# JeffWang987/MVSTER

Hardware: AMD Instinct MI355X
Metric: depth-maps/sec (DTU 512×640, 5-view, 4-stage) at 1/2/4/8 MI355X (higher is better)
Workload: dtype f32; 1 GPU; DTU mid 512x640, 5 views, 4-stage cascade 8/8/4/4 hyp, B=1 eval, 1 depth map(s) per step per GPU; launch=hipGraph replay, parallelism=replicas x1, depth_maps_in_flight_per_gpu=2

## Files before the change

mvster_amd/csrc/conv_wino.hip:

```cpp
#include "conv_args.hpp"

namespace mvconv {
namespace {

typedef float f32x2v __attribute__((ext_vector_type(2)));

#ifdef MVSTER_TIMELINE
__device__ unsigned long long* g_wtl = nullptr;
#define MV_WTL(k)                                                                                                       \
    do {                                                                                                                \
        __builtin_amdgcn_sched_barrier(0);                                                                              \
        if (g_wtl && lane == 0 && g < 32)                                                                               \
            g_wtl[(((size_t)(blockIdx.y * gridDim.x + blockIdx.x) * 8 + wave8) * 32 + g) * 4 + (k)] = __builtin_amdgcn_s_memtime(); \
        __builtin_amdgcn_sched_barrier(0);                                                                              \
    } while (0)
#else
#define MV_WTL(k)
#endif

#ifndef MV_WINO_SCALAR_ADDS
#define MV_WINO_SCALAR_ADDS 0
#endif
#if MV_WINO_SCALAR_ADDS
__device__ __forceinline__ f32x2v pk_add(f32x2v a, f32x2v b) {
    float r0, r1;
    asm("v_add_f32 %0, %2, %3\n\tv_add_f32 %1, %4, %5" : "=&v"(r0), "=&v"(r1) : "v"(a[0]), "v"(b[0]), "v"(a[1]), "v"(b[1]));
    return (f32x2v){r0, r1};
}
__device__ __forceinline__ f32x2v pk_sub(f32x2v a, f32x2v b) {
    float r0, r1;
    asm("v_sub_f32 %0, %2, %3\n\tv_sub_f32 %1, %4, %5" : "=&v"(r0), "=&v"(r1) : "v"(a[0]), "v"(b[0]), "v"(a[1]), "v"(b[1]));
    return (f32x2v){r0, r1};
}
#else
__device__ __forceinline__ f32x2v pk_add(f32x2v a, f32x2v b) {
    f32x2v r;
    asm("v_pk_add_f32 %0, %1, %2" : "=v"(r) : "v"(a), "v"(b));
    return r;
}
__device__ __forceinline__ f32x2v pk_sub(f32x2v a, f32x2v b) {
    f32x2v r;
    asm("v_pk_add_f32 %0, %1, %2 neg_lo:[0,1] neg_hi:[0,1]" : "=v"(r) : "v"(a), "v"(b));
    return r;
}
#endif
struct Q4 {
    f32x2v lo, hi;
};
__device__ __forceinline__ Q4 operator+(const Q4& a, const Q4& b) { return {pk_add(a.lo, b.lo), pk_add(a.hi, b.hi)}; }
__device__ __forceinline__ Q4 operator-(const Q4& a, const Q4& b) { return {pk_sub(a.lo, b.lo), pk_sub(a.hi, b.hi)}; }
__device__ __forceinline__ float elem(const Q4& a, int j) { return j < 2 ? a.lo[j] : a.hi[j - 2]; }

template <int NT, int NCH, bool WREG, bool SKIP>
__global__ void __launch_bounds__(256) conv_wino_kernel(ConvArgs a, PersArgs p) {
    using G = PersGeom<4, 3, 1, 1>;
    constexpr int TY = G::TY, PW = G::PW, PLANE = G::PLANE, NBLK = G::NBLK, RS = G::ROWSLOTS;
    constexpr int BUF = NCH * 2 * PLANE;
    constexpr int NI = NCH * 2 * NBLK;
    constexpr int NIW = (NI + 3) / 4;
    constexpr int CIN = NCH * 16;
    extern __shared__ __attribute__((aligned(16))) float lds_raw[];
    f32x4v* const lds = reinterpret_cast<f32x4v*>(lds_raw);
    f32x4v* const scratch = lds + 2 * BUF;
    f32x4v* const wl = scratch + 64;

    const int lane = threadIdx.x & 63;
    const int wave = __builtin_amdgcn_readfirstlane(threadIdx.x >> 6);
    const int lm = lane & 15, lq = lane >> 4;
    const int nt0 = blockIdx.y * NT;
    const __amdgpu_buffer_rsrc_t in_rsrc =
        __builtin_amdgcn_make_buffer_rsrc(const_cast<float*>(a.in), (short)0, (int)a.in_bytes, 0x00020000);

    unsigned dbase[NIW];
    int dpos[NIW];
#pragma unroll
    for (int n = 0; n < NIW; ++n) {
        const int i = wave + 4 * n;
        const int c = i / (2 * NBLK), r = i - c * 2 * NBLK, pl = r / NBLK, blk = r - pl * NBLK;
        const int s = blk * 64 + lane;
        const int q1 = s & 1, pix = s >> 1;
        const int py = pix / PW, ps = pix - py * PW;
        const int px = ps < G::PWH ? 2 * ps : 2 * (ps - G::PWH) + 1;
        const bool valid = i < NI && py < G::ROWS;
        dpos[n] = px | (py << 8);
        dbase[n] = valid ? (unsigned)((py * a.Wi + px) * (CIN * 4) + (c * 16 + pl * 8 + q1 * 4) * 4) : 0x80000000u;
    }
    auto decode_tile = [&](unsigned tile) -> TilePos {
        TilePos t;
        auto div = [&](unsigned n, int k) -> unsigned { return ((__umulhi(n, p.mul[k]) >> p.shr[k]) & ~p.one[k]) | (n & p.one[k]); };
        unsigned q = div(tile, 0);
        t.tx0 = (int)(tile - q * p.tiles_x) * 32;
        unsigned q2 = div(q, 1);
        t.ty0 = (int)(q - q2 * p.tiles_y) * TY;
        const unsigned q3 = div(q2, 2);
        t.zo = (int)(q2 - q3 * (unsigned)a.Do);
        t.b = (int)q3;
        return t;
    };
    auto dma_tile = [&](const TilePos& t, int buf, bool live) {
        const int iy0 = t.ty0 - a.ph[0], ix0 = t.tx0 - a.pw[0];
        const unsigned origin = (unsigned)((((t.b * a.Di + t.zo) * a.Hi + iy0) * a.Wi + ix0) * (CIN * 4));
        const unsigned wi = live ? (unsigned)a.Wi : 0u;
        f32x4v* const dst0 = lds + buf * BUF;
#pragma unroll
        for (int n = 0; n < NIW; ++n) {
            const int i = wave + 4 * n;
            const int ix = ix0 + (dpos[n] & 255), iy = iy0 + (dpos[n] >> 8);
// ... 23 lines not shown
            const int s = i / NT, nt = i - s * NT;
            const unsigned off = (unsigned)((s * wstep + (long)(nt0 + nt) * 256) * 4) + lane * 16;
            f32x4v* const dst = wl + i * 64;
            __builtin_amdgcn_raw_ptr_buffer_load_lds(w_rsrc, (lds_void*)dst, 16, off, 0, 0, 0);
        }
    }
    f32x4v scv[NT], shv[NT];
#pragma unroll
    for (int nt = 0; nt < NT; ++nt) {
        const int n0 = (nt0 + nt) * 16 + lq * 4;
        scv[nt] = *reinterpret_cast<const f32x4v*>(a.scale + n0);
        shv[nt] = *reinterpret_cast<const f32x4v*>(a.shift + n0);
    }
    const int abase = 2 * wave * RS + 2 * lm + (lq >> 1) * PLANE + (lq & 1);
    const __amdgpu_buffer_rsrc_t out_rsrc =
        __builtin_amdgcn_make_buffer_rsrc(a.out, (short)0, (int)p.out_bytes, 0x00020000);
    const __amdgpu_buffer_rsrc_t skip_rsrc = __builtin_amdgcn_make_buffer_rsrc(
        const_cast<float*>(SKIP ? a.skip : a.in), (short)0, SKIP ? (int)p.out_bytes : 0, 0x00020000);
    const unsigned obase = (unsigned)((2 * wave * a.Wo + 2 * lm) * a.cout + nt0 * 16 + lq * 4) * 4u;
    const unsigned opix = (unsigned)a.cout * 4u, orow = (unsigned)a.Wo * opix;

    __syncthreads();

    for (int it = 0; tile < p.ntiles; tile += nwg, ++it) {
        const int cur = it & 1;
        const TilePos here = pos;
        const unsigned oorigin = (unsigned)((((here.b * a.Do + here.zo) * a.Ho + here.ty0) * a.Wo + here.tx0) * a.cout) * 4u;
        unsigned ooff[2][2];
        f32x4v skv[2][2][NT];
#pragma unroll
        for (int i = 0; i < 2; ++i)
#pragma unroll
            for (int j = 0; j < 2; ++j) {
                const bool ok = here.ty0 + 2 * wave + i < a.Ho && here.tx0 + 2 * lm + j < a.Wo;
                ooff[i][j] = ok ? obase + oorigin + i * orow + j * opix : 0x80000000u;
#pragma unroll
                for (int nt = 0; nt < NT; ++nt)
                    skv[i][j][nt] = SKIP ? __builtin_bit_cast(f32x4v, __builtin_amdgcn_raw_buffer_load_b128(skip_rsrc, ooff[i][j] + nt * 64, 0, 0))
                                         : (f32x4v){0.f, 0.f, 0.f, 0.f};
            }
        const bool has_next = tile + nwg < p.ntiles;
        pos = decode_tile(has_next ? tile + nwg : tile);
        dma_tile(pos, cur ^ 1, has_next);
        __builtin_amdgcn_sched_barrier(0);

        f32x4v acc[16][NT];
#pragma unroll
        for (int q = 0; q < 16; ++q)
#pragma unroll
            for (int nt = 0; nt < NT; ++nt) acc[q][nt] = (f32x4v){0.f, 0.f, 0.f, 0.f};
        const f32x4v* patch = lds + cur * BUF + abase;
#pragma unroll
        for (int c = 0; c < NCH; ++c) {
            Q4 d[4][4], V[4][4];
#pragma unroll
            for (int r = 0; r < 4; ++r)
#pragma unroll
                for (int x = 0; x < 4; ++x) {
                    const f32x4v v = patch[c * 2 * PLANE + r * RS + (x & 1) * (G::PWH * 2) + (x >> 1) * 2];
                    d[r][x] = {{v[0], v[1]}, {v[2], v[3]}};
                }
#pragma unroll
            for (int x = 0; x < 4; ++x) {
                const Q4 t0 = d[0][x] - d[2][x], t1 = d[1][x] + d[2][x], t2 = d[2][x] - d[1][x], t3 = d[1][x] - d[3][x];
                d[0][x] = t0;
                d[1][x] = t1;
                d[2][x] = t2;
                d[3][x] = t3;
            }
#pragma unroll
            for (int r = 0; r < 4; ++r) {
                V[r][0] = d[r][0] - d[r][2];
                V[r][1] = d[r][1] + d[r][2];
                V[r][2] = d[r][2] - d[r][1];
                V[r][3] = d[r][1] - d[r][3];
            }
            __builtin_amdgcn_sched_barrier(0);
            asm volatile("s_nop 3" ::: "memory");
            __builtin_amdgcn_sched_barrier(0);
#pragma unroll
            for (int j = 0; j < 4; ++j)
#pragma unroll
                for (int q = 0; q < 16; ++q)
#pragma unroll
                    for (int nt = 0; nt < NT; ++nt) {
                        const f32x4v u = WREG ? wreg[(q * NCH + c) * NT + nt] : wl[((q * NCH + c) * NT + nt) * 64 + lane];
                        acc[q][nt] = __builtin_amdgcn_mfma_f32_16x16x4f32(u[j], elem(V[q >> 2][q & 3], j), acc[q][nt], 0, 0, 0);
                    }
            __builtin_amdgcn_sched_barrier(0);
        }
        asm volatile("s_nop 15\n\ts_nop 7" ::: "memory");
        __builtin_amdgcn_sched_barrier(0);
        const float floor_v = a.relu ? 0.0f : -__builtin_inff();
#pragma unroll
        for (int nt = 0; nt < NT; ++nt) {
            Q4 m[16], t[2][4];
#pragma unroll
            for (int q = 0; q < 16; ++q) m[q] = {{acc[q][nt][0], acc[q][nt][1]}, {acc[q][nt][2], acc[q][nt][3]}};
#pragma unroll
            for (int x = 0; x < 4; ++x) {
                t[0][x] = m[0 + x] + m[4 + x] + m[8 + x];
                t[1][x] = m[4 + x] - (m[8 + x] + m[12 + x]);
            }
#pragma unroll
            for (int i = 0; i < 2; ++i) {
                Q4 y[2];
                y[0] = t[i][0] + t[i][1] + t[i][2];
                y[1] = t[i][1] - (t[i][2] + t[i][3]);
#pragma unroll
                for (int j = 0; j < 2; ++j) {
                    f32x4v v = {y[j].lo[0], y[j].lo[1], y[j].hi[0], y[j].hi[1]};
#pragma unroll
                    for (int e = 0; e < 4; ++e) {
                        v[e] = fmaxf(fmaf(v[e], scv[nt][e], shv[nt][e]), floor_v);
                        if (SKIP) v[e] += skv[i][j][nt][e];
                    }
                    __builtin_amdgcn_raw_buffer_store_b128(__builtin_bit_cast(u32x4v, v), out_rsrc, ooff[i][j] + nt * 64, 0, MV_STORE_AUX);
                }
            }
        }
        asm volatile("s_waitcnt vmcnt(%0)" ::"n"(4 * NT) : "memory");
        __builtin_amdgcn_s_waitcnt(0xc07f);
        __builtin_amdgcn_s_barrier();
    }
}

template <int NT, int NCH, bool WREG, bool SKIP>
int launch_wino(const ConvArgs& a, int wpc, hipStream_t s) {
    using G = PersGeom<4, 3, 1, 1>;
    const size_t lds = (size_t)(2 * NCH * 2 * G::PLANE + 64 + (WREG ? 0 : 16 * NCH * NT * 64)) * 16;
    if (lds > 160 * 1024) return MVSTER_ERR_UNSUPPORTED;
    auto kern = conv_wino_kernel<NT, NCH, WREG, SKIP>;
    static unsigned long attr_done = 0;
    if (lds > 64 * 1024 && !allow_big_lds(reinterpret_cast<const void*>(kern), attr_done)) return MVSTER_ERR_LAUNCH;
    const int ncu = num_cus();
    if (ncu <= 0) return MVSTER_ERR_LAUNCH;
    PersArgs p;
    if (!fill_pers_args(a, G::TY, p)) return MVSTER_ERR_UNSUPPORTED;
    const long ntiles = p.ntiles;
    const int by_lds = (int)((160 * 1024) / lds);
    int per_cu = wpc > 0 ? wpc : 2;
    if (per_cu > by_lds) per_cu = by_lds;
    if (per_cu < 1) per_cu = 1;
    const int ny = a.ntile_total / NT;
    long gmax = (long)ncu * per_cu / ny;
    if (gmax < 1) gmax = 1;
    const long rounds = (ntiles + gmax - 1) / gmax;
    const long gx = (ntiles + rounds - 1) / rounds;
    MV_NOTE_KERNEL("conv_wino_kernel<%d, %d, %s, %s>", NT, NCH, WREG ? "true" : "false", SKIP ? "true" : "false");
    hipLaunchKernelGGL(kern, dim3((unsigned)gx, ny, 1), dim3(256), lds, s, a, p);
    return mv_check_launch();
}

struct RingGeom {
    static constexpr int TY = 8, PWH = 17, PH = 10;
    static constexpr int ROWSLOTS = PWH * 4;
    static constexpr int USED = PH * ROWSLOTS;
    static constexpr int NBLK = (USED + 63) / 64;
    static constexpr int PLANE = ((NBLK * 64 + 7) & ~7) + 4;
    static constexpr int SLICE = 2 * PLANE;
};

struct RingStep {
    unsigned tile;
    int kz, c, kz_hi;
    TilePos pos;
    bool live;
};

template <int NCH, int KD, bool SKIP, int MODE>
__global__ void __launch_bounds__(512) conv_wino_ring_kernel(ConvArgs a, PersArgs p) {
    constexpr bool SPLITN = MODE == 1;
    constexpr int NT = MODE == 2 ? 2 : 1;
    constexpr int NTW = MODE == 0 ? 1 : 2;
    constexpr bool AHEAD = NT == 1;
    using G = RingGeom;
    constexpr int TY = G::TY, PLANE = G::PLANE, NBLK = G::NBLK, RS = G::ROWSLOTS, SLICE = G::SLICE;
    constexpr int NLW = SPLITN ? 8 : 4;
    constexpr int NIW = (NBLK + NLW / 2 - 1) / (NLW / 2);
    constexpr int NUW = 16 * NTW / NLW;
    constexpr int CIN = NCH * 16;
    constexpr int UST = 16 * NTW * 64;
    constexpr bool URES = KD * NCH * NTW <= 4;
    constexpr int USLOTS = URES ? KD * NCH : 2;
    extern __shared__ __attribute__((aligned(16))) float lds_raw[];
    f32x4v* const ring = reinterpret_cast<f32x4v*>(lds_raw);
    f32x4v* const uring = ring + 4 * SLICE;
    f32x4v* const scratch = uring + USLOTS * UST;

    const int lane = threadIdx.x & 63;
    const int wave8 = __builtin_amdgcn_readfirstlane(threadIdx.x >> 6);
    const int half = wave8 >> 2, wave = wave8 & 3;
    const bool loads = SPLITN || half == 1;
    const int lw = SPLITN ? wave8 : wave;
    const int lm = lane & 15, lq = lane >> 4;
    const int nt0 = blockIdx.y * NTW;
    const int ntw = SPLITN ? half : 0;
    const long wstep = (long)a.ntile_total * 256;
    auto in_rsrc = [&](int k) -> __amdgpu_buffer_rsrc_t {
        return __builtin_amdgcn_make_buffer_rsrc(const_cast<float*>(a.in) - 256 * k, (short)0, (int)(a.in_bytes + 1024u * k), 0x00020000);
    };
    auto w_rsrc = [&](int k) -> __amdgpu_buffer_rsrc_t {
        return __builtin_amdgcn_make_buffer_rsrc(const_cast<float*>(a.wpk) - 256 * k, (short)0,
                                                 (int)(KD * 16 * NCH * wstep * 4 + 1024 * k), 0x00020000);
    };

    static_assert((NLW / 2) * NIW >= NBLK, "the waves of one plane cover its blocks");
    const int lpl = lw / (NLW / 2), lblk0 = (lw % (NLW / 2)) * NIW;
    auto decode_piece = [&](int n, int ln, unsigned& db, int& dp) {
        const int pl = lpl, blk = lblk0 + n;
        const int s = blk * 64 + ln;
        const int q1 = s & 1;
        int t = s >> 1;
        const int xh = t % G::PWH;
        t /= G::PWH;
        const int py = t >> 1, px = 2 * xh + (t & 1);
        const bool valid = blk < NBLK && py < G::PH;
        dp = px | (py << 8);
        db = valid ? (unsigned)((py * a.Wi + px) * (CIN * 4) + (pl * 8 + q1 * 4) * 4) : 0x80000000u;
    };
    unsigned dbase[SPLITN ? NIW : 1];
    int dpos[SPLITN ? NIW : 1];
    if (SPLITN) {
#pragma unroll
// ... 68 lines not shown
            const int ix = r.ix0 + (dp & 255), iy = r.iy0 + (dp >> 8);
            const bool ok = (unsigned)iy < (unsigned)a.Hi && (unsigned)ix < r.wi;
            const unsigned off = ok ? db + r.origin : 0x80000000u;
            switch (n & 3) {
                case 0: __builtin_amdgcn_raw_ptr_buffer_load_lds(rs, (lds_void*)dst, 16, off, 0, IMM[0], 0); break;
                case 1: __builtin_amdgcn_raw_ptr_buffer_load_lds(rs, (lds_void*)dst, 16, off, 0, IMM[1], 0); break;
                case 2: __builtin_amdgcn_raw_ptr_buffer_load_lds(rs, (lds_void*)dst, 16, off, 0, IMM[2], 0); break;
                default: __builtin_amdgcn_raw_ptr_buffer_load_lds(rs, (lds_void*)dst, 16, off, 0, IMM[3], 0); break;
            }
        }
    };
    struct WeightReq {
        unsigned base;
        f32x4v* dst0;
    };
    auto weight_req = [&](const RingStep& st, int slot) -> WeightReq {
        WeightReq r;
        r.base = st.live ? (unsigned)(((long)(st.kz * 16 * NCH + st.c) * wstep + (long)nt0 * 256) * 4) : 0x80000000u;
        r.dst0 = uring + slot * UST;
        return r;
    };
    const unsigned wlane = lane * 16;
    static_assert(NUW <= 8, "two M0 values per weight request");
    auto weight_piece = [&](const WeightReq& r, int m) {
        const int u = lw * NUW + m;
        const int q = u / NTW, nt = u - q * NTW;
        const unsigned so = r.base + (unsigned)(((long)q * NCH * wstep + nt * 256) * 4);
        f32x4v* const dst = r.dst0 + (lw * NUW + (m & ~3)) * 64;
        const __amdgpu_buffer_rsrc_t rs = w_rsrc(m & 3);
        switch (m & 3) {
            case 0: __builtin_amdgcn_raw_ptr_buffer_load_lds(rs, (lds_void*)dst, 16, wlane, so, 0, 0); break;
            case 1: __builtin_amdgcn_raw_ptr_buffer_load_lds(rs, (lds_void*)dst, 16, wlane, so, 1024, 0); break;
            case 2: __builtin_amdgcn_raw_ptr_buffer_load_lds(rs, (lds_void*)dst, 16, wlane, so, 2048, 0); break;
            default: __builtin_amdgcn_raw_ptr_buffer_load_lds(rs, (lds_void*)dst, 16, wlane, so, 3072, 0); break;
        }
    };

    f32x4v scv[NT], shv[NT];
#pragma unroll
    for (int nt = 0; nt < NT; ++nt) {
        const int n0 = (nt0 + ntw + nt) * 16 + lq * 4;
        scv[nt] = *reinterpret_cast<const f32x4v*>(a.scale + n0);
        shv[nt] = *reinterpret_cast<const f32x4v*>(a.shift + n0);
    }
    const int abase = 2 * wave * RS + 2 * lm + (lq >> 1) * PLANE + (lq & 1);
    const __amdgpu_buffer_rsrc_t out_rsrc =
        __builtin_amdgcn_make_buffer_rsrc(a.out, (short)0, (int)p.out_bytes, 0x00020000);
    const __amdgpu_buffer_rsrc_t skip_rsrc = __builtin_amdgcn_make_buffer_rsrc(
        const_cast<float*>(SKIP ? a.skip : a.in), (short)0, SKIP ? (int)p.out_bytes : 0, 0x00020000);
    const unsigned obase = (unsigned)((2 * wave * a.Wo + 2 * lm) * a.cout + (nt0 + ntw) * 16 + lq * 4) * 4u;
    const unsigned opix = (unsigned)a.cout * 4u, orow = (unsigned)a.Wo * opix;
    const float floor_v = a.relu ? 0.0f : -__builtin_inff();

    Q4 d[4][4], V[4][4];
    auto read_block = [&](int slot) {
        const f32x4v* patch = ring + slot * SLICE + abase;
#pragma unroll
        for (int r = 0; r < 4; ++r)
#pragma unroll
            for (int x = 0; x < 4; ++x) {
                const f32x4v v = patch[r * RS + (x & 1) * (G::PWH * 2) + (x >> 1) * 2];
                d[r][x] = {{v[0], v[1]}, {v[2], v[3]}};
            }
    };
    auto transform_block = [&]() {
#pragma unroll
        for (int x = 0; x < 4; ++x) {
            const Q4 t0 = d[0][x] - d[2][x], t1 = d[1][x] + d[2][x], t2 = d[2][x] - d[1][x], t3 = d[1][x] - d[3][x];
            d[0][x] = t0;
            d[1][x] = t1;
            d[2][x] = t2;
            d[3][x] = t3;
        }
#pragma unroll
        for (int r = 0; r < 4; ++r) {
            V[r][0] = d[r][0] - d[r][2];
            V[r][1] = d[r][1] + d[r][2];
            V[r][2] = d[r][2] - d[r][1];
            V[r][3] = d[r][1] - d[r][3];
        }
    };

    RingStep s0 = first_step(xcd_remap(blockIdx.x, nwg));
    RingStep s1 = next_step(s0), s2 = next_step(s1), s3 = next_step(s2);
    if (loads) {
        unsigned db0[NIW];
        int dp0[NIW];
#pragma unroll
        for (int n = 0; n < NIW; ++n) decode_piece(n, lane, db0[n], dp0[n]);
        const RingStep* const first[3] = {&s0, &s1, &s2};
#pragma unroll
        for (int k = 0; k < 3; ++k) {
            const SliceReq r = slice_req(*first[k], k);
#pragma unroll
            for (int n = 0; n < NIW; ++n) slice_piece(r, n, db0[n], dp0[n]);
        }
        if (URES) {
#pragma unroll
            for (int kz = 0; kz < KD; ++kz)
#pragma unroll
                for (int c = 0; c < NCH; ++c) {
                    RingStep st = s0;
                    st.live = true;
                    st.kz = kz;
                    st.c = c;
                    const WeightReq wq = weight_req(st, kz * NCH + c);
#pragma unroll
                    for (int m = 0; m < NUW; ++m) weight_piece(wq, m);
                }
        } else {
            const WeightReq w0 = weight_req(s0, 0);
#pragma unroll
            for (int m = 0; m < NUW; ++m) weight_piece(w0, m);
        }
    }
    __syncthreads();
    if (!SPLITN && half == 1) {
        unsigned dbl[NIW];
        int dpl[NIW];
#pragma unroll
        for (int n = 0; n < NIW; ++n) decode_piece(n, lane, dbl[n], dpl[n]);
        for (int g = 0; s0.live; ++g) {
            MV_WTL(0);
            if (!URES) {
                const WeightReq wr = weight_req(s1, (g + 1) & 1);
#pragma unroll
                for (int m = 0; m < NUW; ++m) weight_piece(wr, m);
            }
            const SliceReq sr = slice_req(s3, (g + 3) & 3);
#pragma unroll
            for (int n = 0; n < NIW; ++n) slice_piece(sr, n, dbl[n], dpl[n]);
            MV_WTL(1);
            asm volatile("s_waitcnt vmcnt(%0)" ::"n"(NIW) : "memory");
            MV_WTL(2);
            __builtin_amdgcn_s_barrier();
            MV_WTL(3);
            s0 = s1;
            s1 = s2;
            s2 = s3;
            s3 = next_step(s3);
        }
        return;
    }
    f32x4v acc[16][NT];
#pragma unroll
    for (int q = 0; q < 16; ++q)
#pragma unroll
        for (int nt = 0; nt < NT; ++nt) acc[q][nt] = (f32x4v){0.f, 0.f, 0.f, 0.f};
    read_block(0);
    transform_block();

    for (int g = 0; s0.live; ++g) {
        const bool last = is_last(s0);
        MV_WTL(0);
        {
            unsigned ooff[2][2];
            f32x4v skv[2][2][NT];
            if (last) {
                const TilePos& here = s0.pos;
                const unsigned oorigin = (unsigned)((((here.b * a.Do + here.zo) * a.Ho + here.ty0) * a.Wo + here.tx0) * a.cout) * 4u;
#pragma unroll
                for (int i = 0; i < 2; ++i)
#pragma unroll
                    for (int j = 0; j < 2; ++j) {
                        const bool ok = here.ty0 + 2 * wave + i < a.Ho && here.tx0 + 2 * lm + j < a.Wo;
                        ooff[i][j] = ok ? obase + oorigin + i * orow + j * opix : 0x80000000u;
#pragma unroll
                        for (int nt = 0; nt < NT; ++nt)
                            skv[i][j][nt] = (SKIP && AHEAD) ? __builtin_bit_cast(f32x4v, __builtin_amdgcn_raw_buffer_load_b128(skip_rsrc, ooff[i][j] + nt * 64, 0, 0))
                                                            : (f32x4v){0.f, 0.f, 0.f, 0.f};
                    }
            }
            const WeightReq wr = weight_req(s1, (g + 1) & 1);
            const SliceReq sr = slice_req(s3, (g + 3) & 3);
            const f32x4v* const nextp = ring + ((g + 1) & 3) * SLICE + abase;
            __builtin_amdgcn_sched_barrier(0);
            {
                const f32x4v* const us = uring + (URES ? s0.kz * NCH + s0.c : g & 1) * UST + ntw * 64 + lane;
                f32x4v ub[2][4][NT];
                auto load_u = [&](int grp, f32x4v (&dst)[4][NT]) {
#pragma unroll
                    for (int qq = 0; qq < 4; ++qq)
#pragma unroll
                        for (int nt = 0; nt < NT; ++nt) dst[qq][nt] = us[((grp * 4 + qq) * NTW + nt) * 64];
                };
                constexpr int NUL = URES ? 0 : NUW;
                constexpr int NP = SPLITN ? NUL + NIW : 0;
                load_u(0, ub[0]);
#pragma unroll
                for (int grp = 0; grp < 4; ++grp) {
                    if (grp < 3) load_u(grp + 1, ub[(grp + 1) & 1]);
#pragma unroll
                    for (int j = 0; j < 4; ++j)
#pragma unroll
                        for (int qq = 0; qq < 4; ++qq)
#pragma unroll
                            for (int nt = 0; nt < NT; ++nt)
                                acc[grp * 4 + qq][nt] = __builtin_amdgcn_mfma_f32_16x16x4f32(ub[grp & 1][qq][nt][j], elem(V[grp][qq], j),
                                                                                             acc[grp * 4 + qq][nt], 0, 0, 0);
                    __builtin_amdgcn_sched_barrier(0);
#pragma unroll
                    for (int k = grp * 2; k < grp * 2 + 2 && k < NP; ++k) {
                        if (k < NUL) {
                            weight_piece(wr, k);
                        } else {
                            slice_piece(sr, k - NUL, dbase[k - NUL], dpos[k - NUL]);
                        }
                    }
                    if (AHEAD) {
#pragma unroll
                        for (int x = 0; x < 4; ++x) {
                            const f32x4v v = nextp[grp * RS + (x & 1) * (G::PWH * 2) + (x >> 1) * 2];
                            d[grp][x] = {{v[0], v[1]}, {v[2], v[3]}};
                        }
                    }
                    __builtin_amdgcn_sched_barrier(0);
                }
            }
            MV_WTL(1);
            __builtin_amdgcn_sched_barrier(0);
            asm volatile("s_nop 15\n\ts_nop 7" ::: "memory");
            __builtin_amdgcn_sched_barrier(0);
            if (last) {
                if (SKIP && !AHEAD) {
#pragma unroll
                    for (int i = 0; i < 2; ++i)
#pragma unroll
                        for (int j = 0; j < 2; ++j)
#pragma unroll
                            for (int nt = 0; nt < NT; ++nt)
                                skv[i][j][nt] = __builtin_bit_cast(f32x4v, __builtin_amdgcn_raw_buffer_load_b128(skip_rsrc, ooff[i][j] + nt * 64, 0, 0));
                }
#pragma unroll
                for (int nt = 0; nt < NT; ++nt) {
                    Q4 m[16], t[2][4];
#pragma unroll
                    for (int q = 0; q < 16; ++q) m[q] = {{acc[q][nt][0], acc[q][nt][1]}, {acc[q][nt][2], acc[q][nt][3]}};
#pragma unroll
                    for (int x = 0; x < 4; ++x) {
                        t[0][x] = m[0 + x] + m[4 + x] + m[8 + x];
                        t[1][x] = m[4 + x] - (m[8 + x] + m[12 + x]);
                    }
#pragma unroll
                    for (int i = 0; i < 2; ++i) {
                        Q4 y[2];
                        y[0] = t[i][0] + t[i][1] + t[i][2];
                        y[1] = t[i][1] - (t[i][2] + t[i][3]);
#pragma unroll
                        for (int j = 0; j < 2; ++j) {
                            f32x4v v = {y[j].lo[0], y[j].lo[1], y[j].hi[0], y[j].hi[1]};
#pragma unroll
                            for (int e = 0; e < 4; ++e) {
                                v[e] = fmaxf(fmaf(v[e], scv[nt][e], shv[nt][e]), floor_v);
                                if (SKIP) v[e] += skv[i][j][nt][e];
                            }
                            __builtin_amdgcn_raw_buffer_store_b128(__builtin_bit_cast(u32x4v, v), out_rsrc, ooff[i][j] + nt * 64, 0, MV_STORE_AUX);
                        }
                    }
                }
#pragma unroll
                for (int q = 0; q < 16; ++q)
#pragma unroll
                    for (int nt = 0; nt < NT; ++nt) acc[q][nt] = (f32x4v){0.f, 0.f, 0.f, 0.f};
            }
            __builtin_amdgcn_sched_barrier(0);
            if (!AHEAD) read_block((g + 1) & 3);
            transform_block();
            MV_WTL(2);
            __builtin_amdgcn_sched_barrier(0);
            if (SPLITN) {
                if (last) {
                    asm volatile("s_waitcnt vmcnt(%0)" ::"n"(NIW + 4 * NT) : "memory");
                } else {
                    asm volatile("s_waitcnt vmcnt(%0)" ::"n"(NIW) : "memory");
                }
            }
        }
        __builtin_amdgcn_s_waitcnt(0xc07f);
        __builtin_amdgcn_s_barrier();
        MV_WTL(3);
        s0 = s1;
        s1 = s2;
        s2 = s3;
        s3 = next_step(s3);
    }
}

template <int NCH, int KD, bool SKIP, int MODE>
int launch_wino_ring(const ConvArgs& a, hipStream_t s) {
    using G = RingGeom;
    constexpr int NT = MODE == 0 ? 1 : 2;
    constexpr int USLOTS = KD * NCH * NT <= 4 ? KD * NCH : 2;
    const size_t lds = (size_t)(4 * G::SLICE + USLOTS * 16 * NT * 64 + 64) * 16;
    if (lds > 160 * 1024) return MVSTER_ERR_UNSUPPORTED;
    auto kern = conv_wino_ring_kernel<NCH, KD, SKIP, MODE>;
    static unsigned long attr_done = 0;
    if (!allow_big_lds(reinterpret_cast<const void*>(kern), attr_done)) return MVSTER_ERR_LAUNCH;
    const int ncu = num_cus();
    if (ncu <= 0) return MVSTER_ERR_LAUNCH;
    PersArgs p;
    if (!fill_pers_args(a, G::TY, p)) return MVSTER_ERR_UNSUPPORTED;
    if ((long)KD * 16 * NCH * a.ntile_total * 1024 >= (1L << 31)) return MVSTER_ERR_UNSUPPORTED;
    const long ntiles = p.ntiles;
    const int ny = a.ntile_total / NT;
    long gmax = (long)ncu / ny;
    if (gmax < 1) gmax = 1;
    const long rounds = (ntiles + gmax - 1) / gmax;
    const long gx = (ntiles + rounds - 1) / rounds;
    MV_NOTE_KERNEL("conv_wino_ring_kernel<%d, %d, %s, %d>", NCH, KD, SKIP ? "true" : "false", MODE);
    hipLaunchKernelGGL(kern, dim3((unsigned)gx, ny, 1), dim3(512), lds, s, a, p);
    return mv_check_launch();
}

template <int NCH, bool SKIP>
__global__ void __launch_bounds__(512) conv_wino_pair_kernel(ConvArgs a, PersArgs p) {
    using G = RingGeom;
    constexpr int KD = 3, NS = 2;
    constexpr int TY = G::TY, PLANE = G::PLANE, NBLK = G::NBLK, RS = G::ROWSLOTS, SLICE = G::SLICE;
    constexpr int NLW = 4;
    constexpr int NIW = (NBLK + NLW / 2 - 1) / (NLW / 2);
    constexpr int CIN = NCH * 16;
    constexpr int UBLK = 16 * 64;
    constexpr bool URES = KD * NCH <= 3;
    constexpr int UST = URES ? UBLK : NS * UBLK;
    constexpr int USLOTS = URES ? KD * NCH : 2;
    constexpr int NUW = NS * 16 / NLW;
    extern __shared__ __attribute__((aligned(16))) float lds_raw[];
    f32x4v* const ring = reinterpret_cast<f32x4v*>(lds_raw);
    f32x4v* const uring = ring + 4 * SLICE;
    f32x4v* const scratch = uring + USLOTS * UST;

    const int lane = threadIdx.x & 63;
    const int wave8 = __builtin_amdgcn_readfirstlane(threadIdx.x >> 6);
    const int half = wave8 >> 2, wave = wave8 & 3;
    const int lm = lane & 15, lq = lane >> 4;
    const int nt0 = blockIdx.y;
    const long wstep = (long)a.ntile_total * 256;
    const int dop = a.Do >> 1;
    auto in_rsrc = [&](int k) -> __amdgpu_buffer_rsrc_t {
        return __builtin_amdgcn_make_buffer_rsrc(const_cast<float*>(a.in) - 256 * k, (short)0, (int)(a.in_bytes + 1024u * k), 0x00020000);
    };
    auto w_rsrc = [&](int k) -> __amdgpu_buffer_rsrc_t {
        return __builtin_amdgcn_make_buffer_rsrc(const_cast<float*>(a.wpk) - 256 * k, (short)0,
                                                 (int)(KD * 16 * NCH * wstep * 4 + 1024 * k), 0x00020000);
    };
    const int lpl = wave / (NLW / 2), lblk0 = (wave % (NLW / 2)) * NIW;
    auto decode_piece = [&](int n, int ln, unsigned& db, int& dp) {
        const int blk = lblk0 + n;
        const int s = blk * 64 + ln;
        const int q1 = s & 1;
        int t = s >> 1;
        const int xh = t % G::PWH;
        t /= G::PWH;
        const int py = t >> 1, px = 2 * xh + (t & 1);
        const bool valid = blk < NBLK && py < G::PH;
        dp = px | (py << 8);
        db = valid ? (unsigned)((py * a.Wi + px) * (CIN * 4) + (lpl * 8 + q1 * 4) * 4) : 0x80000000u;
    };
    auto decode_tile = [&](unsigned tile) -> TilePos {
        TilePos t;
        auto div = [&](unsigned n, int k) -> unsigned { return ((__umulhi(n, p.mul[k]) >> p.shr[k]) & ~p.one[k]) | (n & p.one[k]); };
        unsigned q = div(tile, 0);
// ... 309 lines not shown
struct PackWinoDesc {
    const float* w;
    float* wpk;
    long s_n, s_c, s_z, s_y, s_x;
    int cout, cin_raw, cin, kd, flip, ntile;
    int first_block, pad_;
};

__device__ __forceinline__ void pack_wino_element(const PackWinoDesc& d, long idx) {
    const int cin = d.cin, kd = d.kd, ntile = d.ntile, flip = d.flip;
    const long total = (long)kd * 16 * cin * ntile * 16;
    if (idx >= total) return;
    const int j = (int)(idx & 3), lanei = (int)((idx >> 2) & 63);
    const long rest = idx >> 8;
    const int t = (int)(rest % ntile);
    const int kstep = (int)(rest / ntile);
    const int k = kstep * 16 + (lanei >> 4) * 4 + j;
    const int n = t * 16 + (lanei & 15);
    const int qz = k / cin, ci = k - qz * cin;
    const int kz = qz >> 4, q = qz & 15;
    float u = 0.f;
    if (n < d.cout && ci < d.cin_raw) {
        const int xi = q >> 2, nu = q & 3;
        const float Gm[4][3] = {{1.f, 0.f, 0.f}, {0.5f, 0.5f, 0.5f}, {0.5f, -0.5f, 0.5f}, {0.f, 0.f, 1.f}};
        const float* g = d.w + n * d.s_n + ci * d.s_c + (flip ? kd - 1 - kz : kz) * d.s_z;
        float rowv[3];
#pragma unroll
        for (int x = 0; x < 3; ++x) {
            float acc = 0.f;
#pragma unroll
            for (int y = 0; y < 3; ++y) {
                const int yy = flip ? 2 - y : y, xx = flip ? 2 - x : x;
                acc = fmaf(Gm[xi][y], g[yy * d.s_y + xx * d.s_x], acc);
            }
            rowv[x] = acc;
        }
        u = fmaf(Gm[nu][0], rowv[0], fmaf(Gm[nu][1], rowv[1], Gm[nu][2] * rowv[2]));
    }
    d.wpk[idx] = u;
}

__global__ void pack_wino_kernel(PackWinoDesc d) { pack_wino_element(d, (long)blockIdx.x * blockDim.x + threadIdx.x); }

__global__ void __launch_bounds__(256) pack_wino_batch_kernel(const PackWinoDesc* __restrict__ descs, int ndesc) {
    int lo = 0, hi = ndesc - 1;
    while (lo < hi) {
        const int mid = (lo + hi + 1) >> 1;
        if (descs[mid].first_block <= (int)blockIdx.x) lo = mid; else hi = mid - 1;
    }
    const PackWinoDesc d = descs[lo];
    pack_wino_element(d, (long)((int)blockIdx.x - d.first_block) * 256 + threadIdx.x);
}

}

int dispatch_wino(const ConvArgs& a, int nt, int wpc, bool ring, hipStream_t s) {
    if (a.nclass != 1 || a.osd != 1 || a.osh != 1 || a.osw != 1 || a.skip_mode > 1 || a.prob_w || a.cout % 16 != 0 ||
        a.sh != 1 || a.sw != 1 || a.sd != 1 || a.kh[0] != 3 || a.kw[0] != 3 || a.ph[0] != 1 || a.pw[0] != 1 ||
        nt < 1 || a.ntile_total % nt != 0 || a.cin % 16 != 0)
        return MVSTER_ERR_UNSUPPORTED;
    const int nch = a.cin / 16, kd = a.kd[0];
    if (!(kd == 1 && a.pd[0] == 0) && !(kd == 3 && a.pd[0] == 1)) return MVSTER_ERR_UNSUPPORTED;
    if (ring) {
        if (nt == 1 && wpc == 3) {
            if (kd != 3) return MVSTER_ERR_UNSUPPORTED;
            if (nch == 1) return a.skip_mode == 1 ? launch_wino_pair<1, true>(a, s) : launch_wino_pair<1, false>(a, s);
            if (nch == 2) return a.skip_mode == 1 ? launch_wino_pair<2, true>(a, s) : launch_wino_pair<2, false>(a, s);
            return MVSTER_ERR_UNSUPPORTED;
        }
        const int mode = nt == 1 ? 0 : (wpc == 1 ? 2 : 1);
#define MV_R(MODE_, NCH_, KD_)                                                                      \
    if (mode == MODE_ && nch == NCH_ && kd == KD_)                                                  \
        return a.skip_mode == 1 ? launch_wino_ring<NCH_, KD_, true, MODE_>(a, s) : launch_wino_ring<NCH_, KD_, false, MODE_>(a, s);
        MV_R(0, 1, 3) MV_R(0, 2, 3) MV_R(1, 2, 3) MV_R(2, 2, 3) MV_R(0, 4, 3) MV_R(1, 4, 3) MV_R(2, 4, 3)
        MV_R(0, 4, 1) MV_R(1, 4, 1) MV_R(2, 4, 1) MV_R(0, 2, 1) MV_R(1, 2, 1) MV_R(2, 2, 1) MV_R(0, 1, 1) MV_R(2, 1, 1)
#undef MV_R
        return MVSTER_ERR_UNSUPPORTED;
    }
    if (kd != 1) return MVSTER_ERR_UNSUPPORTED;
#define MV_W(NT_, NCH_, WREG_)                                                                      \
    if (nt == NT_ && nch == NCH_)                                                                   \
        return a.skip_mode == 1 ? launch_wino<NT_, NCH_, WREG_, true>(a, wpc, s) : launch_wino<NT_, NCH_, WREG_, false>(a, wpc, s);
    MV_W(1, 1, true)
    MV_W(2, 1, true)
    MV_W(2, 2, false)
    MV_W(1, 2, false)
#undef MV_W
    return MVSTER_ERR_UNSUPPORTED;
}

}

#ifdef MVSTER_TIMELINE
extern "C" int mvster_debug_wino_timeline(void* buf) {
    return hipMemcpyToSymbol(HIP_SYMBOL(mvconv::g_wtl), &buf, sizeof(buf)) == hipSuccess ? MVSTER_OK : MVSTER_ERR_LAUNCH;
}
#endif

extern "C" int mvster_pack_wino_weights(const float* w, float* wpk, int cout, int cin_raw, int cin_pad, int kd, long s_n, long s_c,
                                        long s_z, long s_y, long s_x, int flip, void* stream) {
    if (!w || !wpk) return MVSTER_ERR_NULL;
    if (cout < 1 || cin_raw < 1 || cin_pad < cin_raw || cin_pad % 16 != 0 || (kd != 1 && kd != 3)) return MVSTER_ERR_SHAPE;
    const int ntile = (cout + 15) / 16;
    const long total = (long)kd * 16 * cin_pad * ntile * 16;
    mvconv::PackWinoDesc d{w, wpk, s_n, s_c, s_z, s_y, s_x, cout, cin_raw, cin_pad, kd, flip, ntile, 0, 0};
    hipLaunchKernelGGL(mvconv::pack_wino_kernel, dim3((unsigned)((total + 255) / 256)), dim3(256), 0, (hipStream_t)stream, d);
    return mv_check_launch();
}

extern "C" int mvster_pack_wino_batch(const void* descs, int ndesc, int total_blocks, void* stream) {
    if (!descs) return MVSTER_ERR_NULL;
    if (ndesc < 1 || total_blocks < 1) return MVSTER_ERR_SHAPE;
    static_assert(sizeof(mvconv::PackWinoDesc) == 88, "PackWinoDesc layout");
    hipLaunchKernelGGL(mvconv::pack_wino_batch_kernel, dim3((unsigned)total_blocks), dim3(256), 0, (hipStream_t)stream,
                       (const mvconv::PackWinoDesc*)descs, ndesc);
    return mv_check_launch();
}
```

Before: 1151 depth-maps/s.

## Add software-pipelined Winograd ring path interleaving next-slice transform with MFMAs

Adds a non-serial variant of the Winograd ring kernel for mode 0, NCH=2, KD=3. It holds the transformed input tile in scalar registers for two parities and interleaves the LDS reads and input transform of the next slice between the MFMAs of the current slice. Non-serial variants also use scalar adds instead of packed adds and drop the s_nop padding, aiming to hide transform latency behind matrix math. The cost is higher register pressure. Other shapes keep the old serial form by default, and the alternative form can only be selected through order bits when probes are compiled in.

Measured after the change: 1148 depth-maps/s. No clear change (-0.2%).

```diff
diff --git a/mvster_amd/csrc/conv_wino.hip b/mvster_amd/csrc/conv_wino.hip
--- a/mvster_amd/csrc/conv_wino.hip
+++ b/mvster_amd/csrc/conv_wino.hip
@@ -18,21 +18,6 @@
 #define MV_WTL(k)
 #endif
 
-#ifndef MV_WINO_SCALAR_ADDS
-#define MV_WINO_SCALAR_ADDS 0
-#endif
-#if MV_WINO_SCALAR_ADDS
-__device__ __forceinline__ f32x2v pk_add(f32x2v a, f32x2v b) {
-    float r0, r1;
-    asm("v_add_f32 %0, %2, %3\n\tv_add_f32 %1, %4, %5" : "=&v"(r0), "=&v"(r1) : "v"(a[0]), "v"(b[0]), "v"(a[1]), "v"(b[1]));
-    return (f32x2v){r0, r1};
-}
-__device__ __forceinline__ f32x2v pk_sub(f32x2v a, f32x2v b) {
-    float r0, r1;
-    asm("v_sub_f32 %0, %2, %3\n\tv_sub_f32 %1, %4, %5" : "=&v"(r0), "=&v"(r1) : "v"(a[0]), "v"(b[0]), "v"(a[1]), "v"(b[1]));
-    return (f32x2v){r0, r1};
-}
-#else
 __device__ __forceinline__ f32x2v pk_add(f32x2v a, f32x2v b) {
     f32x2v r;
     asm("v_pk_add_f32 %0, %1, %2" : "=v"(r) : "v"(a), "v"(b));
@@ -43,16 +28,40 @@
     asm("v_pk_add_f32 %0, %1, %2 neg_lo:[0,1] neg_hi:[0,1]" : "=v"(r) : "v"(a), "v"(b));
     return r;
 }
-#endif
 struct Q4 {
     f32x2v lo, hi;
 };
 __device__ __forceinline__ Q4 operator+(const Q4& a, const Q4& b) { return {pk_add(a.lo, b.lo), pk_add(a.hi, b.hi)}; }
 __device__ __forceinline__ Q4 operator-(const Q4& a, const Q4& b) { return {pk_sub(a.lo, b.lo), pk_sub(a.hi, b.hi)}; }
 __device__ __forceinline__ float elem(const Q4& a, int j) { return j < 2 ? a.lo[j] : a.hi[j - 2]; }
-
-template <int NT, int NCH, bool WREG, bool SKIP>
+__device__ __forceinline__ Q4 from4(const Q4*, const f32x4v& v) { return {{v[0], v[1]}, {v[2], v[3]}}; }
+
+struct S4 {
+    float v[4];
+};
+__device__ __forceinline__ S4 operator+(const S4& a, const S4& b) { return {{a.v[0] + b.v[0], a.v[1] + b.v[1], a.v[2] + b.v[2], a.v[3] + b.v[3]}}; }
+__device__ __forceinline__ S4 operator-(const S4& a, const S4& b) { return {{a.v[0] - b.v[0], a.v[1] - b.v[1], a.v[2] - b.v[2], a.v[3] - b.v[3]}}; }
+__device__ __forceinline__ float elem(const S4& a, int j) { return a.v[j]; }
+__device__ __forceinline__ S4 from4(const S4*, const f32x4v& v) { return {{v[0], v[1], v[2], v[3]}}; }
+template <bool SERIAL>
+struct WinoVec {
+    using type = S4;
+};
+template <>
+struct WinoVec<true> {
+    using type = Q4;
+};
+
+constexpr bool wino_ring_serial(int mode, int nch, int kd) { return !(mode == 0 && nch == 2 && kd == 3); }
+#if defined(MVSTER_PROBES) || defined(MVSTER_TIMELINE)
+#define MV_WINO_SERIAL_FORMS 1
+#else
+#define MV_WINO_SERIAL_FORMS 0
+#endif
+
+template <int NT, int NCH, bool WREG, bool SKIP, bool SERIAL>
 __global__ void __launch_bounds__(256) conv_wino_kernel(ConvArgs a, PersArgs p) {
+    using T4 = typename WinoVec<SERIAL>::type;
     using G = PersGeom<4, 3, 1, 1>;
     constexpr int TY = G::TY, PW = G::PW, PLANE = G::PLANE, NBLK = G::NBLK, RS = G::ROWSLOTS;
     constexpr int BUF = NCH * 2 * PLANE;
@@ -182,17 +191,17 @@
         const f32x4v* patch = lds + cur * BUF + abase;
 #pragma unroll
         for (int c = 0; c < NCH; ++c) {
-            Q4 d[4][4], V[4][4];
+            T4 d[4][4], V[4][4];
 #pragma unroll
             for (int r = 0; r < 4; ++r)
 #pragma unroll
                 for (int x = 0; x < 4; ++x) {
                     const f32x4v v = patch[c * 2 * PLANE + r * RS + (x & 1) * (G::PWH * 2) + (x >> 1) * 2];
-                    d[r][x] = {{v[0], v[1]}, {v[2], v[3]}};
+                    d[r][x] = from4((T4*)nullptr, v);
                 }
 #pragma unroll
             for (int x = 0; x < 4; ++x) {
-                const Q4 t0 = d[0][x] - d[2][x], t1 = d[1][x] + d[2][x], t2 = d[2][x] - d[1][x], t3 = d[1][x] - d[3][x];
+                const T4 t0 = d[0][x] - d[2][x], t1 = d[1][x] + d[2][x], t2 = d[2][x] - d[1][x], t3 = d[1][x] - d[3][x];
                 d[0][x] = t0;
                 d[1][x] = t1;
                 d[2][x] = t2;
@@ -206,7 +215,7 @@
                 V[r][3] = d[r][1] - d[r][3];
             }
             __builtin_amdgcn_sched_barrier(0);
-            asm volatile("s_nop 3" ::: "memory");
+            if (SERIAL) asm volatile("s_nop 3" ::: "memory");
             __builtin_amdgcn_sched_barrier(0);
 #pragma unroll
             for (int j = 0; j < 4; ++j)
@@ -219,14 +228,14 @@
                     }
             __builtin_amdgcn_sched_barrier(0);
         }
-        asm volatile("s_nop 15\n\ts_nop 7" ::: "memory");
+        if (SERIAL) asm volatile("s_nop 15\n\ts_nop 7" ::: "memory");
         __builtin_amdgcn_sched_barrier(0);
         const float floor_v = a.relu ? 0.0f : -__builtin_inff();
 #pragma unroll
         for (int nt = 0; nt < NT; ++nt) {
-            Q4 m[16], t[2][4];
-#pragma unroll
-            for (int q = 0; q < 16; ++q) m[q] = {{acc[q][nt][0], acc[q][nt][1]}, {acc[q][nt][2], acc[q][nt][3]}};
+            T4 m[16], t[2][4];
+#pragma unroll
+            for (int q = 0; q < 16; ++q) m[q] = from4((T4*)nullptr, acc[q][nt]);
 #pragma unroll
             for (int x = 0; x < 4; ++x) {
                 t[0][x] = m[0 + x] + m[4 + x] + m[8 + x];
@@ -234,12 +243,12 @@
             }
 #pragma unroll
             for (int i = 0; i < 2; ++i) {
-                Q4 y[2];
+                T4 y[2];
                 y[0] = t[i][0] + t[i][1] + t[i][2];
                 y[1] = t[i][1] - (t[i][2] + t[i][3]);
 #pragma unroll
                 for (int j = 0; j < 2; ++j) {
-                    f32x4v v = {y[j].lo[0], y[j].lo[1], y[j].hi[0], y[j].hi[1]};
+                    f32x4v v = {elem(y[j], 0), elem(y[j], 1), elem(y[j], 2), elem(y[j], 3)};
 #pragma unroll
                     for (int e = 0; e < 4; ++e) {
                         v[e] = fmaxf(fmaf(v[e], scv[nt][e], shv[nt][e]), floor_v);
@@ -255,12 +264,12 @@
     }
 }
 
-template <int NT, int NCH, bool WREG, bool SKIP>
+template <int NT, int NCH, bool WREG, bool SKIP, bool SERIAL>
 int launch_wino(const ConvArgs& a, int wpc, hipStream_t s) {
     using G = PersGeom<4, 3, 1, 1>;
     const size_t lds = (size_t)(2 * NCH * 2 * G::PLANE + 64 + (WREG ? 0 : 16 * NCH * NT * 64)) * 16;
     if (lds > 160 * 1024) return MVSTER_ERR_UNSUPPORTED;
-    auto kern = conv_wino_kernel<NT, NCH, WREG, SKIP>;
+    auto kern = conv_wino_kernel<NT, NCH, WREG, SKIP, SERIAL>;
     static unsigned long attr_done = 0;
     if (lds > 64 * 1024 && !allow_big_lds(reinterpret_cast<const void*>(kern), attr_done)) return MVSTER_ERR_LAUNCH;
     const int ncu = num_cus();
@@ -277,7 +286,7 @@
     if (gmax < 1) gmax = 1;
     const long rounds = (ntiles + gmax - 1) / gmax;
     const long gx = (ntiles + rounds - 1) / rounds;
-    MV_NOTE_KERNEL("conv_wino_kernel<%d, %d, %s, %s>", NT, NCH, WREG ? "true" : "false", SKIP ? "true" : "false");
+    MV_NOTE_KERNEL("conv_wino_kernel<%d, %d, %s, %s>%s", NT, NCH, WREG ? "true" : "false", SKIP ? "true" : "false", SERIAL ? "" : " pipelined");
     hipLaunchKernelGGL(kern, dim3((unsigned)gx, ny, 1), dim3(256), lds, s, a, p);
     return mv_check_launch();
 }
@@ -298,8 +307,9 @@
     bool live;
 };
 
-template <int NCH, int KD, bool SKIP, int MODE>
+template <int NCH, int KD, bool SKIP, int MODE, bool SERIAL>
 __global__ void __launch_bounds__(512) conv_wino_ring_kernel(ConvArgs a, PersArgs p) {
+    using T4 = typename WinoVec<SERIAL>::type;
     constexpr bool SPLITN = MODE == 1;
     constexpr int NT = MODE == 2 ? 2 : 1;
     constexpr int NTW = MODE == 0 ? 1 : 2;
@@ -474,7 +484,7 @@
     const unsigned opix = (unsigned)a.cout * 4u, orow = (unsigned)a.Wo * opix;
     const float floor_v = a.relu ? 0.0f : -__builtin_inff();
 
-    Q4 d[4][4], V[4][4];
+    T4 d[4][4], V[4][4];
     auto read_block = [&](int slot) {
         const f32x4v* patch = ring + slot * SLICE + abase;
 #pragma unroll
@@ -482,13 +492,13 @@
 #pragma unroll
             for (int x = 0; x < 4; ++x) {
                 const f32x4v v = patch[r * RS + (x & 1) * (G::PWH * 2) + (x >> 1) * 2];
-                d[r][x] = {{v[0], v[1]}, {v[2], v[3]}};
+                d[r][x] = from4((T4*)nullptr, v);
             }
     };
     auto transform_block = [&]() {
 #pragma unroll
         for (int x = 0; x < 4; ++x) {
-            const Q4 t0 = d[0][x] - d[2][x], t1 = d[1][x] + d[2][x], t2 = d[2][x] - d[1][x], t3 = d[1][x] - d[3][x];
+            const T4 t0 = d[0][x] - d[2][x], t1 = d[1][x] + d[2][x], t2 = d[2][x] - d[1][x], t3 = d[1][x] - d[3][x];
             d[0][x] = t0;
             d[1][x] = t1;
             d[2][x] = t2;
@@ -569,6 +579,153 @@
     for (int q = 0; q < 16; ++q)
 #pragma unroll
         for (int nt = 0; nt < NT; ++nt) acc[q][nt] = (f32x4v){0.f, 0.f, 0.f, 0.f};
+    auto finish_tile = [&](const unsigned (&ooff)[2][2], const f32x4v (&skv)[2][2][NT]) {
+#pragma unroll
+        for (int nt = 0; nt < NT; ++nt) {
+            T4 m[16], t[2][4];
+#pragma unroll
+            for (int q = 0; q < 16; ++q) m[q] = from4((T4*)nullptr, acc[q][nt]);
+#pragma unroll
+            for (int x = 0; x < 4; ++x) {
+                t[0][x] = m[0 + x] + m[4 + x] + m[8 + x];
+                t[1][x] = m[4 + x] - (m[8 + x] + m[12 + x]);
+            }
+#pragma unroll
+            for (int i = 0; i < 2; ++i) {
+                T4 y[2];
+                y[0] = t[i][0] + t[i][1] + t[i][2];
+                y[1] = t[i][1] - (t[i][2] + t[i][3]);
+#pragma unroll
+                for (int j = 0; j < 2; ++j) {
+                    f32x4v v = {elem(y[j], 0), elem(y[j], 1), elem(y[j], 2), elem(y[j], 3)};
+#pragma unroll
+                    for (int e = 0; e < 4; ++e) {
+                        v[e] = fmaxf(fmaf(v[e], scv[nt][e], shv[nt][e]), floor_v);
+                        if (SKIP) v[e] += skv[i][j][nt][e];
+                    }
+                    __builtin_amdgcn_raw_buffer_store_b128(__builtin_bit_cast(u32x4v, v), out_rsrc, ooff[i][j] + nt * 64, 0, MV_STORE_AUX);
+                }
+            }
+        }
+#pragma unroll
+        for (int q = 0; q < 16; ++q)
+#pragma unroll
+            for (int nt = 0; nt < NT; ++nt) acc[q][nt] = (f32x4v){0.f, 0.f, 0.f, 0.f};
+    };
+    if constexpr (!SERIAL && MODE == 0) {
+        constexpr bool SKIP_EARLY = KD * NCH == 1;
+        float P[2][4][4][4];
+        auto pass_in_place = [&](float& d0, float& d1, float& d2, float& d3) {
+            const float t1 = d1 + d2;
+            d0 = d0 - d2;
+            d2 = d2 - d1;
+            d3 = d1 - d3;
+            d1 = t1;
+        };
+        auto pass_here = [&](float& d0, float& d1, float& d2, float& d3) {
+            pass_in_place(d0, d1, d2, d3);
+            asm volatile("" : "+v"(d0), "+v"(d1), "+v"(d2), "+v"(d3));
+        };
+        {
+            const f32x4v* patch = ring + abase;
+#pragma unroll
+            for (int r = 0; r < 4; ++r)
+#pragma unroll
+                for (int x = 0; x < 4; ++x) {
+                    const f32x4v v = patch[r * RS + (x & 1) * (G::PWH * 2) + (x >> 1) * 2];
+#pragma unroll
+                    for (int e = 0; e < 4; ++e) P[0][r][x][e] = v[e];
+                }
+#pragma unroll
+            for (int x = 0; x < 4; ++x)
+#pragma unroll
+                for (int e = 0; e < 4; ++e) pass_in_place(P[0][0][x][e], P[0][1][x][e], P[0][2][x][e], P[0][3][x][e]);
+#pragma unroll
+            for (int r = 0; r < 4; ++r)
+#pragma unroll
+                for (int e = 0; e < 4; ++e) pass_in_place(P[0][r][0][e], P[0][r][1][e], P[0][r][2][e], P[0][r][3][e]);
+        }
+        int g = 0;
+        auto step = [&](auto parity) __attribute__((always_inline)) {
+            constexpr int CUR = decltype(parity)::value, NXT = CUR ^ 1;
+            const bool last = is_last(s0);
+            MV_WTL(0);
+            unsigned ooff[2][2];
+            f32x4v skv[2][2][NT];
+            if (last) {
+                const TilePos& here = s0.pos;
+                const unsigned oorigin = (unsigned)((((here.b * a.Do + here.zo) * a.Ho + here.ty0) * a.Wo + here.tx0) * a.cout) * 4u;
+#pragma unroll
+                for (int i = 0; i < 2; ++i)
+#pragma unroll
+                    for (int j = 0; j < 2; ++j) {
+                        const bool ok = here.ty0 + 2 * wave + i < a.Ho && here.tx0 + 2 * lm + j < a.Wo;
+                        ooff[i][j] = ok ? obase + oorigin + i * orow + j * opix : 0x80000000u;
+                        if (SKIP && SKIP_EARLY) skv[i][j][0] = __builtin_bit_cast(f32x4v, __builtin_amdgcn_raw_buffer_load_b128(skip_rsrc, ooff[i][j], 0, 0));
+                    }
+            }
+            const f32x4v* const nextp = ring + ((g + 1) & 3) * SLICE + abase;
+            const f32x4v* const us = uring + (URES ? s0.kz * NCH + s0.c : g & 1) * UST + lane;
+            __builtin_amdgcn_sched_barrier(0);
+            f32x4v ub[2][4];
+#pragma unroll
+            for (int qq = 0; qq < 4; ++qq) ub[0][qq] = us[qq * 64];
+#pragma unroll
+            for (int grp = 0; grp < 4; ++grp) {
+                if (grp < 3) {
+#pragma unroll
+                    for (int qq = 0; qq < 4; ++qq) ub[(grp + 1) & 1][qq] = us[((grp + 1) * 4 + qq) * 64];
+                }
+                __builtin_amdgcn_sched_barrier(0);
+#pragma unroll
+                for (int k = 0; k < 16; ++k) {
+                    const int j = k >> 2, qq = k & 3;
+                    acc[grp * 4 + qq][0] = __builtin_amdgcn_mfma_f32_16x16x4f32(ub[grp & 1][qq][j], P[CUR][grp][qq][j], acc[grp * 4 + qq][0], 0, 0, 0);
+                    if (grp < 2) {
+                        if ((k & 1) == 0) {
+                            const int r = 2 * grp + (k >> 3), x = (k >> 1) & 3;
+                            const f32x4v v = nextp[r * RS + (x & 1) * (G::PWH * 2) + (x >> 1) * 2];
+#pragma unroll
+                            for (int e = 0; e < 4; ++e) P[NXT][r][x][e] = v[e];
+                        }
+                    } else if (grp == 2) {
+                        pass_here(P[NXT][0][k >> 2][k & 3], P[NXT][1][k >> 2][k & 3], P[NXT][2][k >> 2][k & 3], P[NXT][3][k >> 2][k & 3]);
+                    } else {
+                        pass_here(P[NXT][k >> 2][0][k & 3], P[NXT][k >> 2][1][k & 3], P[NXT][k >> 2][2][k & 3], P[NXT][k >> 2][3][k & 3]);
+                    }
+                    __builtin_amdgcn_sched_barrier(0);
+                }
+            }
+            MV_WTL(1);
+            __builtin_amdgcn_sched_barrier(0);
+            if (last) {
+                if (SKIP && !SKIP_EARLY) {
+#pragma unroll
+                    for (int i = 0; i < 2; ++i)
+#pragma unroll
+                        for (int j = 0; j < 2; ++j)
+                            skv[i][j][0] = __builtin_bit_cast(f32x4v, __builtin_amdgcn_raw_buffer_load_b128(skip_rsrc, ooff[i][j], 0, 0));
+                }
+                finish_tile(ooff, skv);
+            }
+            MV_WTL(2);
+            __builtin_amdgcn_sched_barrier(0);
+            __builtin_amdgcn_s_waitcnt(0xc07f);
+            __builtin_amdgcn_s_barrier();
+            MV_WTL(3);
+            s0 = s1;
+            s1 = s2;
+            s2 = s3;
+            s3 = next_step(s3);
+            ++g;
+        };
+        while (s0.live) {
+            step(std::integral_constant<int, 0>{});
+            if (!s0.live) break;
+            step(std::integral_constant<int, 1>{});
+        }
+        return;
+    }
     read_block(0);
     transform_block();
 
@@ -633,7 +790,7 @@
 #pragma unroll
                         for (int x = 0; x < 4; ++x) {
                             const f32x4v v = nextp[grp * RS + (x & 1) * (G::PWH * 2) + (x >> 1) * 2];
-                            d[grp][x] = {{v[0], v[1]}, {v[2], v[3]}};
+                            d[grp][x] = from4((T4*)nullptr, v);
                         }
                     }
                     __builtin_amdgcn_sched_barrier(0);
@@ -641,7 +798,7 @@
             }
             MV_WTL(1);
             __builtin_amdgcn_sched_barrier(0);
-            asm volatile("s_nop 15\n\ts_nop 7" ::: "memory");
+            if (SERIAL) asm volatile("s_nop 15\n\ts_nop 7" ::: "memory");
             __builtin_amdgcn_sched_barrier(0);
             if (last) {
                 if (SKIP && !AHEAD) {
@@ -653,37 +810,7 @@
                             for (int nt = 0; nt < NT; ++nt)
                                 skv[i][j][nt] = __builtin_bit_cast(f32x4v, __builtin_amdgcn_raw_buffer_load_b128(skip_rsrc, ooff[i][j] + nt * 64, 0, 0));
                 }
-#pragma unroll
-                for (int nt = 0; nt < NT; ++nt) {
-                    Q4 m[16], t[2][4];
-#pragma unroll
-                    for (int q = 0; q < 16; ++q) m[q] = {{acc[q][nt][0], acc[q][nt][1]}, {acc[q][nt][2], acc[q][nt][3]}};
-#pragma unroll
-                    for (int x = 0; x < 4; ++x) {
-                        t[0][x] = m[0 + x] + m[4 + x] + m[8 + x];
-                        t[1][x] = m[4 + x] - (m[8 + x] + m[12 + x]);
-                    }
-#pragma unroll
-                    for (int i = 0; i < 2; ++i) {
-                        Q4 y[2];
-                        y[0] = t[i][0] + t[i][1] + t[i][2];
-                        y[1] = t[i][1] - (t[i][2] + t[i][3]);
-#pragma unroll
-                        for (int j = 0; j < 2; ++j) {
-                            f32x4v v = {y[j].lo[0], y[j].lo[1], y[j].hi[0], y[j].hi[1]};
-#pragma unroll
-                            for (int e = 0; e < 4; ++e) {
-                                v[e] = fmaxf(fmaf(v[e], scv[nt][e], shv[nt][e]), floor_v);
-                                if (SKIP) v[e] += skv[i][j][nt][e];
-                            }
-                            __builtin_amdgcn_raw_buffer_store_b128(__builtin_bit_cast(u32x4v, v), out_rsrc, ooff[i][j] + nt * 64, 0, MV_STORE_AUX);
-                        }
-                    }
-                }
-#pragma unroll
-                for (int q = 0; q < 16; ++q)
-#pragma unroll
-                    for (int nt = 0; nt < NT; ++nt) acc[q][nt] = (f32x4v){0.f, 0.f, 0.f, 0.f};
+                finish_tile(ooff, skv);
             }
             __builtin_amdgcn_sched_barrier(0);
             if (!AHEAD) read_block((g + 1) & 3);
@@ -708,14 +835,14 @@
     }
 }
 
-template <int NCH, int KD, bool SKIP, int MODE>
+template <int NCH, int KD, bool SKIP, int MODE, bool SERIAL>
 int launch_wino_ring(const ConvArgs& a, hipStream_t s) {
     using G = RingGeom;
     constexpr int NT = MODE == 0 ? 1 : 2;
     constexpr int USLOTS = KD * NCH * NT <= 4 ? KD * NCH : 2;
     const size_t lds = (size_t)(4 * G::SLICE + USLOTS * 16 * NT * 64 + 64) * 16;
     if (lds > 160 * 1024) return MVSTER_ERR_UNSUPPORTED;
-    auto kern = conv_wino_ring_kernel<NCH, KD, SKIP, MODE>;
+    auto kern = conv_wino_ring_kernel<NCH, KD, SKIP, MODE, SERIAL>;
     static unsigned long attr_done = 0;
     if (!allow_big_lds(reinterpret_cast<const void*>(kern), attr_done)) return MVSTER_ERR_LAUNCH;
     const int ncu = num_cus();
@@ -729,7 +856,8 @@
     if (gmax < 1) gmax = 1;
     const long rounds = (ntiles + gmax - 1) / gmax;
     const long gx = (ntiles + rounds - 1) / rounds;
-    MV_NOTE_KERNEL("conv_wino_ring_kernel<%d, %d, %s, %d>", NCH, KD, SKIP ? "true" : "false", MODE);
+    MV_NOTE_KERNEL("conv_wino_ring_kernel<%d, %d, %s, %d>%s", NCH, KD, SKIP ? "true" : "false", MODE,
+                   SERIAL == wino_ring_serial(MODE, NCH, KD) ? "" : SERIAL ? " serial" : " pipelined");
     hipLaunchKernelGGL(kern, dim3((unsigned)gx, ny, 1), dim3(512), lds, s, a, p);
     return mv_check_launch();
 }
@@ -1145,9 +1273,34 @@
     pack_wino_element(d, (long)((int)blockIdx.x - d.first_block) * 256 + threadIdx.x);
 }
 
+template <int NCH, int KD, int MODE>
+int ring_order(const ConvArgs& a, int order, hipStream_t s) {
+    constexpr bool DEF = wino_ring_serial(MODE, NCH, KD);
+    if (order == 0 || (order == 1) == DEF)
+        return a.skip_mode == 1 ? launch_wino_ring<NCH, KD, true, MODE, DEF>(a, s) : launch_wino_ring<NCH, KD, false, MODE, DEF>(a, s);
+#if MV_WINO_SERIAL_FORMS
+    return a.skip_mode == 1 ? launch_wino_ring<NCH, KD, true, MODE, !DEF>(a, s) : launch_wino_ring<NCH, KD, false, MODE, !DEF>(a, s);
+#else
+    return MVSTER_ERR_UNSUPPORTED;
+#endif
+}
+template <int NT, int NCH, bool WREG>
+int plain_order(const ConvArgs& a, int order, int wpc, hipStream_t s) {
+    if (order != 2)
+        return a.skip_mode == 1 ? launch_wino<NT, NCH, WREG, true, true>(a, wpc, s) : launch_wino<NT, NCH, WREG, false, true>(a, wpc, s);
+#if MV_WINO_SERIAL_FORMS
+    return a.skip_mode == 1 ? launch_wino<NT, NCH, WREG, true, false>(a, wpc, s) : launch_wino<NT, NCH, WREG, false, false>(a, wpc, s);
+#else
+    return MVSTER_ERR_UNSUPPORTED;
+#endif
+}
+
 }
 
 int dispatch_wino(const ConvArgs& a, int nt, int wpc, bool ring, hipStream_t s) {
+    const int order = (wpc >> 4) & 3;
+    wpc &= 15;
+    if (order == 3 || (order != 0 && !MV_WINO_SERIAL_FORMS)) return MVSTER_ERR_UNSUPPORTED;
     if (a.nclass != 1 || a.osd != 1 || a.osh != 1 || a.osw != 1 || a.skip_mode > 1 || a.prob_w || a.cout % 16 != 0 ||
         a.sh != 1 || a.sw != 1 || a.sd != 1 || a.kh[0] != 3 || a.kw[0] != 3 || a.ph[0] != 1 || a.pw[0] != 1 ||
         nt < 1 || a.ntile_total % nt != 0 || a.cin % 16 != 0)
@@ -1164,7 +1317,7 @@
         const int mode = nt == 1 ? 0 : (wpc == 1 ? 2 : 1);
 #define MV_R(MODE_, NCH_, KD_)                                                                      \
     if (mode == MODE_ && nch == NCH_ && kd == KD_)                                                  \
-        return a.skip_mode == 1 ? launch_wino_ring<NCH_, KD_, true, MODE_>(a, s) : launch_wino_ring<NCH_, KD_, false, MODE_>(a, s);
+        return ring_order<NCH_, KD_, MODE_>(a, order, s);
         MV_R(0, 1, 3) MV_R(0, 2, 3) MV_R(1, 2, 3) MV_R(2, 2, 3) MV_R(0, 4, 3) MV_R(1, 4, 3) MV_R(2, 4, 3)
         MV_R(0, 4, 1) MV_R(1, 4, 1) MV_R(2, 4, 1) MV_R(0, 2, 1) MV_R(1, 2, 1) MV_R(2, 2, 1) MV_R(0, 1, 1) MV_R(2, 1, 1)
 #undef MV_R
@@ -1173,7 +1326,7 @@
     if (kd != 1) return MVSTER_ERR_UNSUPPORTED;
 #define MV_W(NT_, NCH_, WREG_)                                                                      \
     if (nt == NT_ && nch == NCH_)                                                                   \
-        return a.skip_mode == 1 ? launch_wino<NT_, NCH_, WREG_, true>(a, wpc, s) : launch_wino<NT_, NCH_, WREG_, false>(a, wpc, s);
+        return plain_order<NT_, NCH_, WREG_>(a, order, wpc, s);
     MV_W(1, 1, true)
     MV_W(2, 1, true)
     MV_W(2, 2, false)
```
